# rpng/R-VIO

Measured on AMD Instinct MI355X. Metric: camera frames/sec (KLT+RANSAC track, IMU propagate, MSCKF update, augment/compose), 200 feat / 10-clone window, higher is better.
Workload: dtype f64 (filter) / u8+i32+f32 (KLT); 1 GPU; cfgB: synthetic EuRoC-shaped 752x480 @20Hz, 200 features, 10-clone window, IMU 200 Hz, single stream, equalizer on (CLAHE 3.0, 5x5), corners from the device detector (GFTT + cornerSubPix); parallelism=single GPU

## Files before the change

r-vio_amd/csrc/filter_kernels.hip:

```cpp
#include <type_traits>
#include "rvio_dev.h"
#include "../../include/rvio_hip.h"
#include "solve9.hip"

#include "literal.h"
__device__ const double kChi2Dev[500] = {
#include "chi2_table.inc"
};

typedef double d4 __attribute__((ext_vector_type(4)));

__device__ __forceinline__ double fast_rcp(double v) {
    double y = __builtin_amdgcn_rcp(v);
    y = fma(fma(-v, y, 1.0), y, y);
    return fma(fma(-v, y, 1.0), y, y);
}
__device__ __forceinline__ void sincos_fast(double x, double* sp, double* cp) {
    if (!(fabs(x) < 1e5)) { sincos(x, sp, cp); return; }
    const double kf = rint(x * 6.36619772367581382433e-01);
    double r = fma(-kf, 1.57079632679489655800e+00, x);
    r = fma(-kf, 6.12323399573676603587e-17, r);
    const int q = (int)kf & 3;
    const double z = r * r;
    double ps = fma(z, 1.58969099521155010221e-10, -2.50507602534068634195e-08);
// ... 1712 lines not shown
        for (int u = 0; u < 22; ++u) {
            const int e = tid + u * 256;
            const int rr = e >> 6, k = e & 63;
            if (rr < 88) { Gl[rr * LS + k] = vg[u]; Ul[rr * LS + k] = vu[u]; }
            const int k2 = e / 88, r2 = e - k2 * 88;
            if (k2 < 64) P1c[r2 * LS + k2] = vp[u];
        }
    }
    __syncthreads();
    const int nt = (d + 15) / 16, npair = nt * (nt + 1) / 2;
    const int pr = blockIdx.x * 4 + wave;
    if (pr >= npair) return;
    int I = 0, rem = pr;
    while (rem >= nt - I) { rem -= nt - I; ++I; }
    const int J = I + rem;
    auto xtile = [&](int i0, int j0) -> d4 {
        const int r = i0 + li, c = j0 + li;
        double a1[16], b1[16], p1[4];
#pragma unroll
        for (int q = 0; q < 4; ++q) { const int row = i0 + lk + 4 * q; p1[q] = (row < d && c < d) ? P1[(size_t)row + (size_t)c * ld] : 0.0; }
#pragma unroll
        for (int u = 0; u < 16; ++u) { const int k = 4 * u + lk; a1[u] = (r < d) ? P1c[r * LS + k] : 0.0; b1[u] = (c < d) ? Gl[c * LS + k] : 0.0; }
        d4 acc = {0, 0, 0, 0}, acc2 = {0, 0, 0, 0};
#pragma unroll
        for (int u = 0; u < 16; ++u) acc = __builtin_amdgcn_mfma_f64_16x16x4f64(a1[u], b1[u], acc, 0, 0, 0);
#pragma unroll
        for (int u = 0; u < 16; ++u) { const int k = 4 * u + lk; a1[u] = (r < d) ? Gl[r * LS + k] : 0.0; b1[u] = (c < d) ? Ul[c * LS + k] : 0.0; }
#pragma unroll
        for (int u = 0; u < 16; ++u) acc2 = __builtin_amdgcn_mfma_f64_16x16x4f64(a1[u], b1[u], acc2, 0, 0, 0);
        d4 out;
#pragma unroll
        for (int q = 0; q < 4; ++q) out[q] = p1[q] - acc[q] + s2 * acc2[q];
        return out;
    };
    const d4 xij = xtile(I * 16, J * 16);
    d4 xji = xij;
    if (I != J) xji = xtile(J * 16, I * 16);
#pragma unroll
    for (int q = 0; q < 4; ++q) tl[wave][lk + 4 * q][li] = xji[q];
    __builtin_amdgcn_wave_barrier();
#pragma unroll
    for (int q = 0; q < 4; ++q) {
        const int rr = lk + 4 * q, row = I * 16 + rr, col = J * 16 + li;
        const double v = .5 * (xij[q] + tl[wave][li][rr]);
        if (row < d && col < d) {
            Pout[(size_t)row + (size_t)col * ld] = v;
            if (I != J) Pout[(size_t)col + (size_t)row * ld] = v;
        }
    }
}

#define JL_LS 61
#define JL_LDS_DOUBLES (3 * 60 * JL_LS + 8 * 16 * JL_LS + 16)
__global__ __launch_bounds__(256) void joseph_lds_kernel(DevCfg cfg, int n, const double* __restrict__ P, const double* __restrict__ W, const double* __restrict__ Ab,
                                                         double* __restrict__ Pout, FilterMeta* __restrict__ meta, const double* __restrict__ x, double* __restrict__ x_out,
                                                         const double* __restrict__ dx_scr, int n_pairs, int dx_nt) {
    if (dx_scr && (int)blockIdx.x >= n_pairs) {
        __shared__ S9DxLds dxl;
        s9_dx_role(cfg, meta, n, Ab, x, P, dx_scr, x_out, dx_nt, (int)blockIdx.x - n_pairs, dxl);
        return;
    }
    extern __shared__ __align__(16) double jl[];
    constexpr int LS = JL_LS;
    double* const Wl = jl;
    double* const Al = Wl + 60 * LS;
    double* const Ccl = Al + 60 * LS;
    double* const PcS = Ccl + 60 * LS;
    double* const Us = PcS + 2 * 16 * LS;
    double* const Gs = Us + 2 * 16 * LS;
    double* const Qs = Gs + 2 * 16 * LS;
    constexpr int SS = 16 * LS;
    const int c6 = 6 * n, d = 24 + c6, ldh = cfg.ldh, ld = cfg.dmax;
    const double s2 = cfg.sigma_im * cfg.sigma_im;
    const int tid = threadIdx.x, lane = tid & 63, wave = tid >> 6, li = lane & 15, lk = lane >> 4;
    DBG_R(blockIdx.x == 0, 3);
    const int nt = (d + 15) / 16;
    int I = 0, rem = blockIdx.x;
    while (rem >= nt - I) { rem -= nt - I; ++I; }
    const int J = I + rem;
    const int r0[2] = {I * 16, J * 16};
    auto r0of = [&](int sidx) { return sidx ? J * 16 : I * 16; };
    DBG_T(20);
    double p0[4] = {0, 0, 0, 0}, p0t[4] = {0, 0, 0, 0};
    if (wave == 0) {
#pragma unroll
        for (int q = 0; q < 4; ++q) {
            const int row = r0[0] + lk + 4 * q, c = r0[1] + li;
            const bool ok = row < d && c < d;
            p0[q] = ok ? P[(size_t)row + (size_t)c * ld] : 0.0;
            p0t[q] = ok ? P[(size_t)c + (size_t)row * ld] : 0.0;
        }
    }
    auto ldz = [](const double* __restrict__ p, size_t i, bool ok) { const double v = p[ok ? i : 0]; return ok ? v : 0.0; };
    double vw[15], va[15], vc[15], vs[8];
#pragma unroll
    for (int u = 0; u < 15; ++u) {
        const int e = tid + u * 256, k = e / 60, j = e - k * 60;
        vw[u] = ldz(W, (size_t)k * ldh + j, e < 3600 && k < c6 && j < c6);
    }
#pragma unroll
    for (int u = 0; u < 8; ++u) {
        const int e = tid + u * 256, sidx = e / 960, ee = e - sidx * 960, k = ee >> 4, rr = ee & 15;
        const int row = r0of(sidx & 1) + rr;
        vs[u] = ldz(P, (size_t)row + (size_t)(24 + k) * ld, e < 1920 && k < c6 && row < d);
    }
#pragma unroll
    for (int u = 0; u < 15; ++u) {
        const int e = tid + u * 256, k = e / 60, j = e - k * 60;
        va[u] = ldz(Ab, (size_t)k * ldh + j, e < 3600 && k < c6 && j < c6);
    }
#pragma unroll
    for (int u = 0; u < 15; ++u) {
        const int e = tid + u * 256, k = e / 60, j = e - k * 60;
        vc[u] = ldz(P, (size_t)(24 + j) + (size_t)(24 + k) * ld, e < 3600 && k < c6 && j < c6);
    }
    for (int e = tid; e < 6 * SS; e += 256) Us[e] = 0.0;
#pragma unroll
    for (int u = 0; u < 15; ++u) {
        const int e = tid + u * 256, k = e / 60, j = e - k * 60;
        if (e < 3600) Wl[k * LS + j] = vw[u];
    }
#pragma unroll
    for (int u = 0; u < 8; ++u) {
        const int e = tid + u * 256, sidx = e / 960, ee = e - sidx * 960, k = ee >> 4, rr = ee & 15;
        if (e < 1920) PcS[(sidx & 1) * SS + rr * LS + k] = vs[u];
    }
    __syncthreads();
    DBG_T(21);
    const int ntj = (c6 + 15) / 16;
    auto strips = [&](const double* X, const double* Ym, bool Yt, double* out, const double* sub) {
        const int t0 = wave, t1 = wave + 4, ntile = 2 * ntj;
        const bool v0 = t0 < ntile, v1 = t1 < ntile;
        const int s0 = min(t0 / ntj, 1), c0 = (t0 % ntj) * 16 + li, s1 = min(t1 / ntj, 1), c1 = (t1 % ntj) * 16 + li;
        double a0[15], b0[15], a1[15], b1[15];
#pragma unroll
        for (int u = 0; u < 15; ++u) {
            const int k = 4 * u + lk;
            a0[u] = X[s0 * SS + li * LS + k];
            b0[u] = Yt ? Ym[c0 * LS + k] : Ym[k * LS + c0];
            a1[u] = X[s1 * SS + li * LS + k];
            b1[u] = Yt ? Ym[c1 * LS + k] : Ym[k * LS + c1];
        }
        d4 acc0 = {0, 0, 0, 0}, acc1 = {0, 0, 0, 0};
#pragma unroll
        for (int u = 0; u < 15; ++u) {
            acc0 = __builtin_amdgcn_mfma_f64_16x16x4f64(a0[u], b0[u], acc0, 0, 0, 0);
            acc1 = __builtin_amdgcn_mfma_f64_16x16x4f64(a1[u], b1[u], acc1, 0, 0, 0);
        }
        const bool st0 = v0 && c0 < 60, st1 = v1 && c1 < 60;
#pragma unroll
        for (int q = 0; q < 4; ++q) {
            const int row = lk + 4 * q;
            if (st0) out[s0 * SS + row * LS + c0] = sub ? (sub[s0 * SS + row * LS + min(c0, 59)] - acc0[q]) : acc0[q];
            if (st1) out[s1 * SS + row * LS + c1] = sub ? (sub[s1 * SS + row * LS + min(c1, 59)] - acc1[q]) : acc1[q];
        }
    };
    strips(PcS, Wl, false, Us, nullptr);
#pragma unroll
    for (int u = 0; u < 15; ++u) {
        const int e = tid + u * 256, k = e / 60, j = e - k * 60;
        if (e < 3600) { Al[k * LS + j] = va[u]; Ccl[j * LS + k] = vc[u]; }
    }
    __syncthreads();
    DBG_T(22);
    strips(Us, Al, false, Gs, nullptr);
    __syncthreads();
    DBG_T(23);
    strips(Gs, Ccl, true, Qs, PcS);
    __syncthreads();
    DBG_T(24);
    double (*const xt)[16][17] = reinterpret_cast<double (*)[16][17]>(Wl);
    const int nprod = (I == J) ? 3 : 6;
    auto product = [&](int pidx) -> d4 {
        const int sa = pidx / 3, sb = sa ^ 1, kind = pidx - 3 * sa;
        const double* Xa = (kind == 1 ? Qs : Gs) + sa * SS;
        const double* Yb = (kind == 0 ? PcS : (kind == 1 ? Gs : Us)) + sb * SS;
        double a1[15], b1[15];
#pragma unroll
        for (int u = 0; u < 15; ++u) { const int k = 4 * u + lk; a1[u] = Xa[li * LS + k]; b1[u] = Yb[li * LS + k]; }
        d4 acc = {0, 0, 0, 0};
#pragma unroll
        for (int u = 0; u < 15; ++u) acc = __builtin_amdgcn_mfma_f64_16x16x4f64(a1[u], b1[u], acc, 0, 0, 0);
        return acc;
    };
    {
        const bool two = wave + 4 < nprod;
        d4 pa = {0, 0, 0, 0}, pb = {0, 0, 0, 0};
        if (wave < nprod) pa = product(wave);
        if (two) pb = product(wave + 4);
#pragma unroll
        for (int q = 0; q < 4; ++q) {
            if (wave < nprod) xt[wave][lk + 4 * q][li] = pa[q];
            if (two) xt[wave + 4][lk + 4 * q][li] = pb[q];
        }
    }
    __syncthreads();
    DBG_T(25);
    if (wave == 0) {
        const int o = (I == J) ? 0 : 3;
#pragma unroll
        for (int q = 0; q < 4; ++q) {
            const int rr = lk + 4 * q, row = I * 16 + rr, col = J * 16 + li;
            const double p1 = p0[q] - xt[0][rr][li];
            const double xij = p1 - xt[1][rr][li] + s2 * xt[2][rr][li];
            const double p1t = p0t[q] - xt[o][li][rr];
            const double xji = p1t - xt[o + 1][li][rr] + s2 * xt[o + 2][li][rr];
            const double v = .5 * (xij + xji);
            if (row < d && col < d) {
                Pout[(size_t)row + (size_t)col * ld] = v;
                if (I != J) Pout[(size_t)col + (size_t)row * ld] = v;
            }
        }
    }
}
```

r-vio_amd/csrc/launch_plan.h:

```cpp
#pragma once
#include <stddef.h>

#if defined(__HIPCC__) || defined(__CUDACC__)
#define LP_HD __host__ __device__
#else
#define LP_HD
#endif

#define RVIO_MAX_LEN 32
#define RVIO_MAX_FEATURES 4096
#define GRAM_MAX_FEATS 2048
#define RVIO_LDS_LIMIT 163840
#define LIT_FEATS 24
#define LIT_RING 32
#ifndef FEAT_T_SMALL
#define FEAT_T_SMALL 128
#endif
#define LIT_STAMPS 5
#define LIT_STAMP_OFF 200

LP_HD inline size_t feat_lds_doubles(int max_len, int ldh, bool tm_in_lds) {
    const int L = max_len, M2 = 2 * L, rho = 2 * L - 2;
    size_t n = (size_t)7 * (L - 1) + (size_t)(L - 1) * 24 + L * 6 + M2 * 3 + (L - 1) * 18 + 3 * M2 + 16;
    n += (size_t)M2 * ldh;
    if (tm_in_lds) n += (size_t)rho * ldh;
    n += (size_t)(rho + 1) * (rho + 1);
    return n;
}
LP_HD inline int trunc_mmax(int max_len) { return 6 * ((max_len + 1) / 2 - 1); }
LP_HD inline size_t trunc_lds_doubles(int max_len) { const size_t m = trunc_mmax(max_len); return m * (m | 1) + m + 8; }
LP_HD inline size_t gram_batch_lds_doubles(int max_len, int ldh) {
    const size_t a = (size_t)(ldh - 1) * ldh, t = trunc_lds_doubles(max_len);
    return a > t ? a : t;
}
LP_HD inline size_t lit_tri(int c6) { return (size_t)c6 * (c6 + 1) / 2 + c6; }
LP_HD inline size_t lit_aux_doubles(int ldh, int rho_max) { return (size_t)LIT_RING * ldh + 4 * (size_t)ldh + 2 * 256 + ldh + (size_t)(LIT_FEATS * rho_max + 1) / 2 + 8; }
LP_HD inline size_t lit_state_doubles(int c6) { return 3 * lit_tri(c6); }
LP_HD inline size_t lit_slab_doubles(int ldh, int rho_max) { return (size_t)(rho_max + 2) * (ldh + 3); }
LP_HD inline size_t lit_rows_doubles(int ldh, int rho_max) { return (size_t)LIT_FEATS * (rho_max + 2) * (ldh + 3) + (size_t)LIT_FEATS * rho_max * ldh; }
LP_HD inline size_t book_lds_bytes(int F, int waves) { return (((size_t)20 * F + 7) & ~(size_t)7) + (size_t)waves * F * 8 + 16; }

LP_HD inline size_t lit_norm_off(int ldh) { return (size_t)ldh * ldh; }
LP_HD inline bool lit_stamp_fits(int ldh) { return (size_t)ldh * ldh + LIT_STAMP_OFF + LIT_STAMPS <= 2 * (size_t)ldh * ldh; }
LP_HD inline size_t lit_stamp_off(int ldh, int k) { return (size_t)ldh * ldh + LIT_STAMP_OFF + k; }
LP_HD inline size_t lit_diag_end(int ldh, bool stamps) {
    size_t e = lit_norm_off(ldh) + (size_t)(ldh - 1);
    if (stamps && lit_stamp_fits(ldh)) { const size_t s = lit_stamp_off(ldh, LIT_STAMPS - 1) + 1; if (s > e) e = s; }
    return e;
}

#define LP_S9CHOL4_BYTES 35976
#define LP_S9CHOL6_BYTES 44424
#define LP_S9SMALL_BYTES 160328
#define LP_PROP3_BYTES 86432
#define LP_JB_TL_DOUBLES (12 * 16 * 17)
#define LP_UGL_BYTES ((2 * 64 * 65 + 88 * 65 + 2 * 16 * 65) * 8)
#define LP_FNL_BYTES ((3 * 88 * 65 + 4 * 16 * 17) * 8)
#define LP_JL_BYTES ((3 * 60 * 61 + 8 * 16 * 61 + 16) * 8)
#define LP_GEMM_T_LDS_BYTES (2 * 64 * 65 * 8)

enum LpKernel {
    LPK_FEAT_BUILD16, LPK_FEAT_BUILD4, LPK_GRAM_REDUCE, LPK_BLOCK_SUM, LPK_LIT_BATCH, LPK_GEMM_T_LDS, LPK_GRAM_BATCH4, LPK_GRAM_BATCH6, LPK_FEAT_PROP,
    LPK_BOOKKEEP_B, LPK_RANSAC_BOOK, LPK_SOLVE9_SMALL, LPK_SOLVE6_1, LPK_SOLVE6_2, LPK_SOLVE6_3, LPK_JOSEPH_BATCH, LPK_UG, LPK_UG_LDS, LPK_FINAL_LDS,
    LPK_JOSEPH_LDS, LPK_COUNT
};
static const char* const kLpKernelName[LPK_COUNT] = {
    "feat_build_kernel<16>", "feat_build_kernel<4>", "gram_reduce_kernel", "block_sum_kernel", "lit_batch_kernel", "gemm_T_lds_kernel",
    "gram_reduce_batch_kernel<4>", "gram_reduce_batch_kernel<6>", "feat_prop_kernel", "bookkeep_b_kernel", "ransac_book_kernel", "solve9_small_kernel",
    "solve6_kernel<1, 8, 8>", "solve6_kernel<2, 12, 8>", "solve6_kernel<2, 16, 8>", "joseph_batch_kernel", "ug_kernel", "ug_lds_kernel", "final_lds_kernel",
    "joseph_lds_kernel"
};

struct LaunchPlan {
    int rc = 0;
    const char* why = nullptr;
    int Fu = 0, ldh = 0, rho_max = 0;
    int feat_threads = 256;
    int n_ic = 2;
    bool chol_queue = false;
    size_t trunc_lds = 0, lit_batch_lds = 0, feat_lds = 0, fprop_lds = 0, gram_batch_lds = 0, book_lds = 0, solve5_lds = 0, jb_lds = 0, ug_lds = 0;
    bool lit_state_global = false, tm_global = false, fuse_ok = false;
    bool lit_ok = false;
    int book_waves = 4;
    bool book_fused = false;
    int solve5_variant = 0, solve7_variant = 0, solve9_nt = 0;
    size_t attr[LPK_COUNT] = {};
};

LP_HD inline size_t lp_max(size_t a, size_t b) { return a > b ? a : b; }
LP_HD inline size_t lp_min(size_t a, size_t b) { return a < b ? a : b; }

inline LaunchPlan launch_plan(int max_len, int n_features, int batch, const size_t* statics) {
    LaunchPlan p;
    const int nmax = max_len - 1;
    p.Fu = (n_features + 1) / 2; p.ldh = 6 * nmax + 1; p.rho_max = 2 * max_len - 2;
    const size_t ldh = p.ldh, c6m = ldh - 1;
    const int F = n_features;
    if (max_len < 3 || max_len > RVIO_MAX_LEN || n_features < 2 || batch < 1) { p.rc = 1; p.why = "invalid configuration"; return p; }
    if (p.Fu > GRAM_MAX_FEATS) { p.rc = 1; p.why = "Tracker.nFeatures too large: at most 4096 (RVIO_MAX_FEATURES; ceil(F/2) hand-over slots <= 2048 in the Gram stage)"; return p; }
    if (batch == 1 && c6m > 96 && c6m <= 192) { p.n_ic = 1; p.chol_queue = true; }
    p.feat_threads = (p.ldh <= 128) ? FEAT_T_SMALL : 256;
    p.lit_ok = p.ldh <= 190 && nmax + 1 <= 40 && p.rho_max < 254 && lit_slab_doubles(p.ldh, p.rho_max) * sizeof(double) <= 144 * 1024;
    p.trunc_lds = trunc_lds_doubles(max_len) * sizeof(double);
    {
        const size_t aux = lit_aux_doubles(p.ldh, p.rho_max) * sizeof(double), st = lit_state_doubles(p.ldh - 1) * sizeof(double);
        const size_t slab = lit_slab_doubles(p.ldh, p.rho_max) * sizeof(double);
        p.lit_state_global = batch > 1 || aux + st > 144 * 1024;
        p.lit_batch_lds = lp_max(aux, slab);
        p.trunc_lds = lp_max(p.trunc_lds, lp_max(p.lit_state_global ? aux : aux + st, lp_min((size_t)4, (size_t)(144 * 1024) / slab) * slab));
    }
    p.feat_lds = feat_lds_doubles(max_len, p.ldh, true) * sizeof(double);
// ... 364 lines not shown
```

r-vio_amd/csrc/rvio_hip.hip:

```cpp
#include <hip/hip_runtime.h>
#include <atomic>
#include <chrono>
#include <dlfcn.h>
#include <cmath>
#include <cstdio>
#include <cstdlib>
#include <cstring>
#include <map>
#include <mutex>
#include <string>
#include <vector>

#include "../../include/rvio_hip.h"
#include "rvio_dev.h"
#include "frontend_dev.h"
#include "filter_kernels.hip"
#include "filter_kernels2.hip"
#include "solve6.hip"
#include "solve7.hip"
#include "solve9.hip"
#include "landmarks.hip"
#include "odom.hip"
#pragma clang fp contract(off)
#include "frontend_kernels.hip"
// ... 827 lines not shown
    if (NT == 8) hipLaunchKernelGGL((solve9_chol_kernel<2, 4>), dim3(1), dim3(1024), 0, st, h->dc, n, Pc, h->S9scr);
    else hipLaunchKernelGGL((solve9_chol_kernel<3, 4>), dim3(1), dim3(1024), 0, st, h->dc, n, Pc, h->S9scr);
}
static void launch_s9_sweep(rvio_hip* h, int NT, const double* Ab) {
    if (NT == 8) hipLaunchKernelGGL((solve9_sweep_kernel<2, 4>), dim3(1), dim3(1024), 0, h->stream, h->dc, Ab, h->S9scr);
    else hipLaunchKernelGGL((solve9_sweep_kernel<3, 4>), dim3(1), dim3(1024), 0, h->stream, h->dc, Ab, h->S9scr);
}
static bool take_chol(rvio_hip* h) {
    if (h->chol_async && hipStreamWaitEvent(h->stream, h->evL, 0) != hipSuccess) { h->chol_async = false; h->chol_ready = false; }
    const bool pre = h->chol_ready || h->chol_async;
    h->chol_ready = false; h->chol_async = false;
    return pre;
}

static void launch_solve(rvio_hip* h, const UpdateForms& f, int n, const double* Ab) {
    const DevCfg& d = h->dc;
    double *xin = h->x[h->cur], *xout = h->x[h->cur ^ 1], *Pc = h->P[h->cur];
    const dim3 gb(1, 1, h->batch);
    const size_t bs = h->slab_bytes;
    const bool roles = f.dx == LPD_ROLES;
    switch (f.solve) {
    case LPS_NONE: break;
    case LPS_SMALL: hipLaunchKernelGGL(solve9_small_kernel, dim3(1), dim3(1024), f.solve_lds.bytes, h->stream, d, h->meta, n, Ab, xin, Pc, h->S9scr, h->W, xout, roles ? h->S9scr + S9_YP_OFF(4) : (double*)nullptr); break;
    case LPS_S9_1_4: hipLaunchKernelGGL((solve9_kernel<1, 4>), gb, dim3(1024), 0, h->stream, d, h->meta, n, Ab, xin, Pc, h->S9scr, h->W, xout, bs, (size_t)0); break;
    case LPS_S9_2_3_PRE: hipLaunchKernelGGL((solve9_kernel<2, 3, true>), gb, dim3(576), 0, h->stream, d, h->meta, n, Ab, xin, Pc, h->S9scr, h->W, xout, bs, (size_t)0, roles ? 1 : 0); break;
    case LPS_S9_2_3: hipLaunchKernelGGL((solve9_kernel<2, 3>), gb, dim3(576), 0, h->stream, d, h->meta, n, Ab, xin, Pc, h->S9scr, h->W, xout, bs, (size_t)0, roles ? 1 : 0); break;
    case LPS_SPLIT: {
        const int NT = f.split_nt, nwg = (NT * NT + 3) / 4;
        if (f.own_chol) launch_s9_chol(h, NT, n, Pc, h->stream);
        hipLaunchKernelGGL(solve9_prod_kernel<0>, dim3(nwg), dim3(256), 0, h->stream, d, n, Ab, h->S9scr, h->W, NT);
        hipLaunchKernelGGL(solve9_prod_kernel<1>, dim3(nwg), dim3(256), 0, h->stream, d, n, Ab, h->S9scr, h->W, NT);
        launch_s9_sweep(h, NT, Ab);
        hipLaunchKernelGGL(solve9_prod_kernel<2>, dim3(nwg), dim3(256), 0, h->stream, d, n, Ab, h->S9scr, h->W, NT);
        hipLaunchKernelGGL(solve9_prod_kernel<3>, dim3(nwg), dim3(256), 0, h->stream, d, n, Ab, h->S9scr, h->W, NT);
        if (f.dx == LPD_KERNEL) hipLaunchKernelGGL(solve9_dx_kernel, dim3(1), dim3(1024), 0, h->stream, d, h->meta, n, Ab, xin, Pc, h->S9scr, h->W, xout, NT);
        break;
    }
    case LPS_SOLVE7: hipLaunchKernelGGL((solve7_kernel<3, 16, 12>), gb, dim3(768), 0, h->stream, d, h->meta, n, Ab, xin, Pc, h->Tbuf, h->W, xout, bs); break;
    case LPS_SOLVE6_1: hipLaunchKernelGGL((solve6_kernel<1, 8, 8>), gb, dim3(512), f.solve_lds.bytes, h->stream, d, h->meta, n, h->Tbuf, Ab, xin, Pc, h->W, xout, bs); break;
    case LPS_SOLVE6_2: hipLaunchKernelGGL((solve6_kernel<2, 12, 8>), gb, dim3(512), f.solve_lds.bytes, h->stream, d, h->meta, n, h->Tbuf, Ab, xin, Pc, h->W, xout, bs); break;
    case LPS_SOLVE6_3: hipLaunchKernelGGL((solve6_kernel<2, 16, 8>), gb, dim3(512), f.solve_lds.bytes, h->stream, d, h->meta, n, h->Tbuf, Ab, xin, Pc, h->W, xout, bs); break;
    }
}

static void launch_ug_final(rvio_hip* h, const UpdateForms& f, int n, const double* Ab, double* Pn, bool ug, bool fin, bool roles) {
    const DevCfg& d = h->dc;
    const int B = h->batch;
    const size_t bs = h->slab_bytes;
    double* Pc = h->P[h->cur];
    const int role_wgs = roles ? f.role_wgs : 0;
    const double *nod = nullptr, *yp = role_wgs ? (const double*)h->S9scr : nod;
    switch (f.joseph) {
    case LPJ_BATCH: hipLaunchKernelGGL(joseph_batch_kernel, dim3(1, 1, B), dim3(JB_THREADS), f.ug_lds.bytes, h->stream, d, n, Pc, h->W, Ab, Pn, bs); break;
    case LPJ_LDS: hipLaunchKernelGGL(joseph_lds_kernel, dim3(f.grid[0] + role_wgs), dim3(256), f.ug_lds.bytes, h->stream, d, n, Pc, h->W, Ab, Pn, h->meta, (const double*)h->x[h->cur], h->x[h->cur ^ 1], yp, f.grid[0], h->plan.solve9_nt); break;
    case LPJ_LDS_PAIR:
        if (ug) hipLaunchKernelGGL(ug_lds_kernel, dim3(f.grid[0]), dim3(256), f.ug_lds.bytes, h->stream, d, n, Pc, h->W, Ab, h->U, h->G, h->Pt1);
        if (fin) hipLaunchKernelGGL(final_lds_kernel, dim3(f.grid[1]), dim3(256), f.fin_lds.bytes, h->stream, d, n, h->Pt1, h->G, h->U, Pn);
        break;
    case LPJ_TILE:
        if (ug) {
            hipLaunchKernelGGL(ug_tile_kernel<0>, dim3(f.grid[0] + role_wgs), dim3(256), 0, h->stream, d, n, Pc, h->W, Ab, h->U, h->G, h->Pt1,
                               h->meta, (const double*)h->x[h->cur], h->x[h->cur ^ 1], yp, h->plan.solve9_nt);
            hipLaunchKernelGGL(ug_tile_kernel<1>, dim3(f.grid[1]), dim3(256), 0, h->stream, d, n, Pc, h->W, Ab, h->U, h->G, h->Pt1, h->meta, nod, (double*)nullptr, nod, 0);
            hipLaunchKernelGGL(ug_tile_kernel<2>, dim3(f.grid[2]), dim3(256), 0, h->stream, d, n, Pc, h->W, Ab, h->U, h->G, h->Pt1, h->meta, nod, (double*)nullptr, nod, 0);
        }
        if (fin) hipLaunchKernelGGL(final_tile_kernel, dim3(f.grid[3]), dim3(256), 0, h->stream, d, n, h->Pt1, h->G, h->U, Pn);
        break;
    case LPJ_STRIPS:
        if (ug) hipLaunchKernelGGL(ug_kernel, dim3(f.grid[0], 1, B), dim3(256), f.ug_lds.bytes, h->stream, d, n, Pc, h->W, Ab, h->U, h->G, h->Pt1, bs);
        if (fin) hipLaunchKernelGGL(final_kernel, dim3(f.grid[1], 1, B), dim3(256), 0, h->stream, d, n, h->Pt1, h->G, h->U, Pn, bs);
        break;
    }
}

static void launch_landmarks(rvio_hip* h, int n, const LmOut& out) {
    const int T = std::min(LM_MAX_T, 64 * ((h->dc.Fu + 63) / 64));
    hipLaunchKernelGGL(landmark_kernel, dim3(1, 1, h->batch), dim3(T), 0, h->stream, h->dc, n, (const double*)h->x[h->cur ^ 1], (const double*)h->x[h->cur],
                       (const int*)h->t.n_feat, (const unsigned char*)h->t.types, (const int*)h->t.len, (const int*)h->acc, (const double*)h->pfinv,
                       h->slab_bytes, h->bin, out, (const CamCal*)h->cal);
}
static dim3 lp_grid(const LpLaunch& l) { return dim3((unsigned)l.gx, (unsigned)l.gy, (unsigned)l.gz); }
static dim3 lp_block(const LpLaunch& l) { return dim3((unsigned)l.threads); }
static void launch_subpix(rvio_hip* h, const FrontForms& f, const DetDev& q, const uint8_t* img, int stride, size_t src_bs, int frame, hipStream_t st) {
    const size_t bs = h->slab_bytes;
    const LpLaunch& l = f.subpix_l;
    switch (f.subpix) {
    case LPSP_NONE: break;
    case LPSP_WIDE_WIN: hipLaunchKernelGGL(subpix_wide_kernel, lp_grid(l), lp_block(l), l.lds, st, img, stride, q, src_bs, bs); break;
    case LPSP_GENERIC: hipLaunchKernelGGL(subpix_generic_kernel, lp_grid(l), lp_block(l), 0, st, img, stride, q, src_bs, bs); break;
    case LPSP_X16: hipLaunchKernelGGL(subpix_kernel16, lp_grid(l), lp_block(l), 0, st, img, stride, q, src_bs, bs); break;
    case LPSP_STOCK: hipLaunchKernelGGL(subpix_kernel, lp_grid(l), lp_block(l), 0, st, img, stride, q, src_bs, bs, frame); break;
    }
}
static int lm_alloc(rvio_hip* h, LmOut* out) {
    const size_t Fu = (size_t)h->dc.Fu;
    auto up = [](size_t b) { return (b + 255) & ~(size_t)255; };
    const size_t o_feat = 256, o_pr = o_feat + up(sizeof(int) * Fu), o_pw = o_pr + up(sizeof(double) * 3 * Fu), bs = o_pw + up(sizeof(double) * 3 * Fu);
    char* p = nullptr;
    HIPCHK(h, hipMalloc((void**)&p, bs * h->batch));
    h->allocs.push_back(p);
    HIPCHK(h, hipMemsetAsync(p, 0, bs * h->batch, h->stream));
    *out = LmOut{(int*)p, (int*)(p + o_feat), (double*)(p + o_pr), (double*)(p + o_pw), bs};
    return RVIO_OK;
}

static int update_global_dev(rvio_hip* h, const double* d_blocks, int world, bool combined) {
    const DevCfg& d = h->dc;
// ... 1300 lines not shown
```

r-vio_amd/csrc/solve9.hip:

```cpp
#pragma once
#include "rvio_dev.h"

typedef double s9_d4 __attribute__((ext_vector_type(4)));
#define S9_TILE 256

__device__ __forceinline__ bool lane_is(int li, int lk, int a, int b) { return li == a && lk == b; }
struct S9Wave {
    double rowb[2][128];
    double tb[16 * 17 + 64 + 192];
};
typedef __attribute__((address_space(3))) double s9_lds_t;
typedef volatile s9_lds_t* s9_vlp;

__device__ __forceinline__ s9_d4 s9_tn(const s9_d4& x, const s9_d4& y, s9_d4 acc) {
    acc = __builtin_amdgcn_mfma_f64_16x16x4f64(x[0], y[0], acc, 0, 0, 0);
    acc = __builtin_amdgcn_mfma_f64_16x16x4f64(x[1], y[1], acc, 0, 0, 0);
    acc = __builtin_amdgcn_mfma_f64_16x16x4f64(x[2], y[2], acc, 0, 0, 0);
    acc = __builtin_amdgcn_mfma_f64_16x16x4f64(x[3], y[3], acc, 0, 0, 0);
    return acc;
}
__device__ __forceinline__ s9_d4 s9_zero() { s9_d4 z = {0.0, 0.0, 0.0, 0.0}; return z; }
__device__ __forceinline__ s9_d4 s9_ldg(const double* t, int lane) {
    s9_d4 v = {t[lane], t[64 + lane], t[128 + lane], t[192 + lane]};
    return v;
}
__device__ __forceinline__ void s9_stg(double* t, int lane, const s9_d4& v) {
    t[lane] = v[0]; t[64 + lane] = v[1]; t[128 + lane] = v[2]; t[192 + lane] = v[3];
}
__device__ __forceinline__ s9_d4 s9_lds(const double* t_, int lane) {
    const s9_lds_t* t = (const s9_lds_t*)t_;
    s9_d4 v = {t[lane], t[64 + lane], t[128 + lane], t[192 + lane]};
    return v;
}
__device__ __forceinline__ void s9_sts(double* t_, int lane, const s9_d4& v) {
    s9_lds_t* t = (s9_lds_t*)t_;
    t[lane] = v[0]; t[64 + lane] = v[1]; t[128 + lane] = v[2]; t[192 + lane] = v[3];
}
__device__ __forceinline__ s9_d4 s9_transpose_tb(const s9_d4& v, double* tb_, int li, int lk) {
    s9_vlp tb = (s9_vlp)tb_;
#pragma unroll
    for (int r = 0; r < 4; ++r) tb[(4 * r + lk) * 17 + li] = v[r];
    s9_d4 t;
#pragma unroll
    for (int r = 0; r < 4; ++r) t[r] = tb[li * 17 + 4 * r + lk];
    return t;
}

__device__ __forceinline__ double s9_rsqrt(double t) {
    double y = __builtin_amdgcn_rsq(t);
    const double h = 0.5 * t;
    y = fma(y, fma(-(h * y), y, 0.5), y);
    y = fma(y, fma(-(h * y), y, 0.5), y);
    return y;
}
__device__ __forceinline__ void s9_factor(s9_d4 m, const double* ref_, double tol, S9Wave* ws, int li, int lk, s9_d4& F, s9_d4& Ft, int& bad) {
    const s9_lds_t* ref = (const s9_lds_t*)ref_;
    const int lane = li + 16 * lk;
    s9_d4 e;
#pragma unroll
    for (int r = 0; r < 4; ++r) e[r] = (4 * r + lk == li) ? 1.0 : 0.0;
#pragma unroll
    for (int b = 0; b < 4; ++b) {
        s9_vlp rb = (s9_vlp)ws->rowb[b & 1];
        rb[lane] = m[b];
        rb[64 + lane] = e[b];
        const double a00 = rb[0 * 16 + 4 * b + 0];
        const double a10 = rb[1 * 16 + 4 * b + 0], a11 = rb[1 * 16 + 4 * b + 1];
        const double a20 = rb[2 * 16 + 4 * b + 0], a21 = rb[2 * 16 + 4 * b + 1], a22 = rb[2 * 16 + 4 * b + 2];
        const double a30 = rb[3 * 16 + 4 * b + 0], a31 = rb[3 * 16 + 4 * b + 1], a32 = rb[3 * 16 + 4 * b + 2], a33 = rb[3 * 16 + 4 * b + 3];
        double Rv[4], Ev[4];
#pragma unroll
        for (int v = 0; v < 4; ++v) { Rv[v] = rb[v * 16 + li]; Ev[v] = rb[64 + v * 16 + li]; }
        double lim[4];
#pragma unroll
        for (int k = 0; k < 4; ++k) lim[k] = ref_ ? tol * ref[4 * b + k] : 0.0;
        auto pivot = [&](double t, int k) {
            const bool ok = t > lim[k] && t > 0.0;
            if (!ok && (ref_ == nullptr || !(t >= -lim[k]))) bad |= 1;
            return ok ? s9_rsqrt(t) : 0.0;
        };
        const double i0 = pivot(a00, 0);
        const double l10 = a10 * i0, l20 = a20 * i0, l30 = a30 * i0;
        const double i1 = pivot(fma(-l10, l10, a11), 1);
        const double l21 = fma(-l20, l10, a21) * i1, l31 = fma(-l30, l10, a31) * i1;
        const double i2 = pivot(fma(-l21, l21, fma(-l20, l20, a22)), 2);
        const double l32 = fma(-l31, l21, fma(-l30, l20, a32)) * i2;
        const double i3 = pivot(fma(-l32, l32, fma(-l31, l31, fma(-l30, l30, a33))), 3);
        const double f00 = i0, f11 = i1, f22 = i2, f33 = i3;
        const double f10 = -(l10 * f00) * i1;
        const double f21 = -(l21 * f11) * i2;
        const double f32 = -(l32 * f22) * i3;
        const double f20 = -fma(l21, f10, l20 * f00) * i2;
        const double f31 = -fma(l32, f21, l31 * f11) * i3;
        const double f30 = -fma(l32, f20, fma(l31, f10, l30 * f00)) * i3;
        const double g0 = lk == 0 ? f00 : lk == 1 ? f10 : lk == 2 ? f20 : f30;
        const double g1 = lk == 0 ? 0.0 : lk == 1 ? f11 : lk == 2 ? f21 : f31;
        const double g2 = lk <= 1 ? 0.0 : lk == 2 ? f22 : f32;
        const double g3 = lk == 3 ? f33 : 0.0;
        const double z = fma(g3, Rv[3], fma(g2, Rv[2], fma(g1, Rv[1], g0 * Rv[0])));
        const double ze = fma(g3, Ev[3], fma(g2, Ev[2], fma(g1, Ev[1], g0 * Ev[0])));
        const double za = (li > 4 * b + 3) ? -z : 0.0;
        m = __builtin_amdgcn_mfma_f64_16x16x4f64(za, z, m, 0, 0, 0);
        e = __builtin_amdgcn_mfma_f64_16x16x4f64(za, ze, e, 0, 0, 0);
        e[b] = ze;
    }
    F = e;
    Ft = s9_transpose_tb(F, ws->tb, li, lk);
}

template <class FX, class FY>
__device__ __forceinline__ s9_d4 s9_gemm(int k0, int k1, FX fx, FY fy) {
    s9_d4 acc = s9_zero();
    if (k0 >= k1) return acc;
    s9_d4 xa = fx(k0), xb = fy(k0);
#pragma unroll 2
    for (int k = k0; k < k1; ++k) {
        s9_d4 na = xa, nb = xb;
        if (k + 1 < k1) { na = fx(k + 1); nb = fy(k + 1); }
        acc = s9_tn(xa, xb, acc);
        xa = na; xb = nb;
    }
    return acc;
// ... 576 lines not shown
    S9Wave ws;
    double b[64], y[64], yp[4][64];
    double dx[24 + 64];
    double part[4 * (24 + 64)];
    int bad;
};
__global__ __launch_bounds__(1024) void solve9_small_kernel(DevCfg cfg, FilterMeta* __restrict__ meta, int n, const double* __restrict__ Ab,
                                                            const double* __restrict__ x, const double* __restrict__ P, const double* __restrict__ scr,
                                                            double* __restrict__ Wout, double* __restrict__ x_out, double* __restrict__ yp_out) {
    constexpr int NT = 4, NTH = 1024;
    extern __shared__ __align__(16) double s9s_dyn[];
    S9SmallLds& sh = *reinterpret_cast<S9SmallLds*>(s9s_dyn);
    const int c6 = 6 * n, d = 24 + c6, ldh = cfg.ldh, ld = cfg.dmax, xd = 26 + 7 * n;
    const int tid = threadIdx.x, lane = tid & 63, wv = __builtin_amdgcn_readfirstlane(tid >> 6), li = lane & 15, lk = lane >> 4;
    const int ti = wv >> 2, tj = wv & 3;
    const int n_good = (int)Ab[(size_t)ldh * (ldh - 1)], n_rows = (int)Ab[(size_t)ldh * (ldh - 1) + 1];
    const bool upd = n_good > 2;
    DBG_R(true, 2);
    if (tid == 0) { meta->n_good = n_good; meta->n_rows = n_rows; meta->updated = upd ? 1 : 0; meta->trunc_at = (int)Ab[(size_t)ldh * (ldh - 1) + 2]; sh.bad = 0; }
    if (!upd) {
        for (int e = tid; e < c6 * c6; e += NTH) Wout[(size_t)(e / c6) * ldh + (e % c6)] = 0.0;
        if (!yp_out) for (int i = tid; i < xd; i += NTH) x_out[i] = x[i];
        return;
    }
    DBG_T(30);
    const double s2 = cfg.sigma_im * cfg.sigma_im;
    auto ld_A = [&](int i, int j) {
        s9_d4 v;
#pragma unroll
        for (int r = 0; r < 4; ++r) {
            const int row = 16 * i + 4 * r + lk, col = 16 * j + li;
            v[r] = (row < c6 && col < c6) ? Ab[(size_t)row * ldh + col] : 0.0;
        }
        return v;
    };
    const s9_d4 a0 = ld_A(ti, tj);
    const bool lowt = ti >= tj;
    s9_d4 l0 = s9_zero(), g0 = s9_zero();
    if (lowt) { l0 = s9_ldg(scr + (size_t)(ti * NT + tj) * S9_TILE, lane); g0 = s9_ldg(scr + (size_t)NT * NT * S9_TILE + (size_t)(tj * NT + ti) * S9_TILE, lane); }
    constexpr int PCN = (88 * 64 + NTH - 1) / NTH;
    double pc[PCN];
#pragma unroll
    for (int u = 0; u < PCN; ++u) {
        const int e = tid + u * NTH, k = e / 88, i = e - k * 88;
        pc[u] = (!yp_out && k < c6 && i < d) ? P[(size_t)i + (size_t)(24 + k) * ld] : 0.0;
    }
    if (tid < 64) sh.b[tid] = (tid < c6) ? Ab[(size_t)tid * ldh + c6] : 0.0;
    if (tid == 0 && scr[(size_t)5 * NT * NT * S9_TILE] != 0.0) sh.bad = 1;
    if (lowt) { s9_sts(sh.L[ti * NT + tj], lane, l0); s9_sts(sh.G[ti * (ti + 1) / 2 + tj], lane, g0); }
    s9_sts(sh.Q[wv], lane, a0);
    __syncthreads();
    DBG_T(32);
    {
        s9_d4 q = s9_zero(), rr = s9_zero();
#pragma unroll
        for (int k = 0; k < NT; ++k) {
            if (k >= tj) q = s9_tn(s9_lds(sh.Q[k * NT + ti], lane), s9_lds(sh.L[k * NT + tj], lane), q);
            if (k >= ti) rr = s9_tn(s9_lds(sh.L[k * NT + ti], lane), s9_lds(sh.Q[k * NT + tj], lane), rr);
        }
        __syncthreads();
        s9_sts(sh.Q[wv], lane, q);
        s9_sts(sh.R[wv], lane, rr);
    }
    __syncthreads();
    DBG_T(33);
    s9_d4 S = s9_zero();
#pragma unroll
    for (int k = 0; k < NT; ++k)
        if (k >= ti) S = s9_tn(s9_lds(sh.L[k * NT + ti], lane), s9_lds(sh.Q[k * NT + tj], lane), S);
    if (ti == tj) {
#pragma unroll
        for (int r = 0; r < 4; ++r) if (4 * r + lk == li) S[r] += s2;
    }
    DBG_T(34);
    int bad = 0;
#pragma unroll 1
    for (int k = 0; k < NT; ++k) {
        double (*rowp)[S9_TILE] = sh.rowp[k & 1];
        if (ti == k) s9_sts(rowp[tj], lane, S);
        __syncthreads();
        s9_d4 F, Ft;
        if (wv == 0) {
            s9_factor(s9_lds(rowp[k], lane), nullptr, 0.0, &sh.ws, li, lk, F, Ft, bad);
            s9_sts(sh.F[0], lane, F);
            s9_sts(sh.F[1], lane, Ft);
        }
        __syncthreads();
        F = s9_lds(sh.F[0], lane);
        if (wv < NT) {
            Ft = s9_lds(sh.F[1], lane);
            s9_sts(sh.Z[wv], lane, s9_tn(Ft, s9_lds(rowp[wv], lane), s9_zero()));
        }
        __syncthreads();
        if (ti == k && tj == k) {
            const s9_d4 dd = s9_tn(F, F, s9_zero());
#pragma unroll
            for (int r = 0; r < 4; ++r) S[r] = -dd[r];
        } else if (ti == k) S = s9_tn(F, s9_lds(sh.Z[tj], lane), s9_zero());
        else if (tj == k) S = s9_tn(s9_lds(sh.Z[ti], lane), F, s9_zero());
        else {
            const s9_d4 Zr = s9_lds(sh.Z[ti], lane);
            s9_d4 nz;
#pragma unroll
            for (int r = 0; r < 4; ++r) nz[r] = -Zr[r];
            S = s9_tn(nz, s9_lds(sh.Z[tj], lane), S);
        }
    }
    {
        s9_d4 v;
#pragma unroll
        for (int r = 0; r < 4; ++r) v[r] = -S[r];
        s9_sts(sh.Q[wv], lane, v);
    }
    __syncthreads();
    DBG_T(35);
    {
        s9_d4 v = s9_zero();
#pragma unroll
        for (int k = 0; k < NT; ++k) v = s9_tn(s9_lds(sh.Q[k * NT + ti], lane), s9_lds(sh.R[k * NT + tj], lane), v);
        s9_sts(sh.L[wv], lane, v);
    }
    __syncthreads();
    DBG_T(36);
    double* pcs = &sh.Q[0][0];
    if (!yp_out) {
#pragma unroll
        for (int u = 0; u < PCN; ++u) { const int e = tid + u * NTH; if (e < 88 * 64) ((s9_lds_t*)pcs)[e] = pc[u]; }
    }
    {
        const double is2 = 1.0 / s2;
        s9_d4 acc = s9_zero();
#pragma unroll
        for (int k = 0; k < NT; ++k)
            if (k <= ti) acc = s9_tn(s9_lds(sh.G[ti * (ti + 1) / 2 + k], lane), s9_lds(sh.L[k * NT + tj], lane), acc);
        double t = 0.0;
#pragma unroll
        for (int r = 0; r < 4; ++r) {
            const int a = 16 * ti + 4 * r + lk, bcol = 16 * tj + li;
            const double w = (((a == bcol) ? 1.0 : 0.0) - acc[r]) * is2;
            if (a < c6 && bcol < c6) Wout[(size_t)bcol * ldh + a] = w;
            t = fma(w, sh.b[a], t);
        }
        t += __shfl_xor(t, 16); t += __shfl_xor(t, 32);
// ... 43 lines not shown
```

Before: 11050 frames/s.

## Widen Joseph LDS kernel to 512 threads and trim solve9 small-kernel syncs

```diff
diff --git a/r-vio_amd/csrc/filter_kernels.hip b/r-vio_amd/csrc/filter_kernels.hip
--- a/r-vio_amd/csrc/filter_kernels.hip
+++ b/r-vio_amd/csrc/filter_kernels.hip
@@ -1788,7 +1788,7 @@
 
 #define JL_LS 61
 #define JL_LDS_DOUBLES (3 * 60 * JL_LS + 8 * 16 * JL_LS + 16)
-__global__ __launch_bounds__(256) void joseph_lds_kernel(DevCfg cfg, int n, const double* __restrict__ P, const double* __restrict__ W, const double* __restrict__ Ab,
+__global__ __launch_bounds__(LP_JL_THREADS) void joseph_lds_kernel(DevCfg cfg, int n, const double* __restrict__ P, const double* __restrict__ W, const double* __restrict__ Ab,
                                                          double* __restrict__ Pout, FilterMeta* __restrict__ meta, const double* __restrict__ x, double* __restrict__ x_out,
                                                          const double* __restrict__ dx_scr, int n_pairs, int dx_nt) {
     if (dx_scr && (int)blockIdx.x >= n_pairs) {
@@ -1797,7 +1797,7 @@
         return;
     }
     extern __shared__ __align__(16) double jl[];
-    constexpr int LS = JL_LS;
+    constexpr int LS = JL_LS, NTH = LP_JL_THREADS;
     double* const Wl = jl;
     double* const Al = Wl + 60 * LS;
     double* const Ccl = Al + 60 * LS;
@@ -1828,73 +1828,67 @@
         }
     }
     auto ldz = [](const double* __restrict__ p, size_t i, bool ok) { const double v = p[ok ? i : 0]; return ok ? v : 0.0; };
-    double vw[15], va[15], vc[15], vs[8];
-#pragma unroll
-    for (int u = 0; u < 15; ++u) {
-        const int e = tid + u * 256, k = e / 60, j = e - k * 60;
+    double vw[8], va[8], vc[8], vs[4];
+#pragma unroll
+    for (int u = 0; u < 8; ++u) {
+        const int e = tid + u * NTH, k = e / 60, j = e - k * 60;
         vw[u] = ldz(W, (size_t)k * ldh + j, e < 3600 && k < c6 && j < c6);
     }
 #pragma unroll
-    for (int u = 0; u < 8; ++u) {
-        const int e = tid + u * 256, sidx = e / 960, ee = e - sidx * 960, k = ee >> 4, rr = ee & 15;
+    for (int u = 0; u < 4; ++u) {
+        const int e = tid + u * NTH, sidx = e / 960, ee = e - sidx * 960, k = ee >> 4, rr = ee & 15;
         const int row = r0of(sidx & 1) + rr;
         vs[u] = ldz(P, (size_t)row + (size_t)(24 + k) * ld, e < 1920 && k < c6 && row < d);
     }
 #pragma unroll
-    for (int u = 0; u < 15; ++u) {
-        const int e = tid + u * 256, k = e / 60, j = e - k * 60;
+    for (int u = 0; u < 8; ++u) {
+        const int e = tid + u * NTH, k = e / 60, j = e - k * 60;
         va[u] = ldz(Ab, (size_t)k * ldh + j, e < 3600 && k < c6 && j < c6);
     }
 #pragma unroll
-    for (int u = 0; u < 15; ++u) {
-        const int e = tid + u * 256, k = e / 60, j = e - k * 60;
+    for (int u = 0; u < 8; ++u) {
+        const int e = tid + u * NTH, k = e / 60, j = e - k * 60;
         vc[u] = ldz(P, (size_t)(24 + j) + (size_t)(24 + k) * ld, e < 3600 && k < c6 && j < c6);
     }
-    for (int e = tid; e < 6 * SS; e += 256) Us[e] = 0.0;
-#pragma unroll
-    for (int u = 0; u < 15; ++u) {
-        const int e = tid + u * 256, k = e / 60, j = e - k * 60;
+    for (int e = tid; e < 6 * SS; e += NTH) Us[e] = 0.0;
+#pragma unroll
+    for (int u = 0; u < 8; ++u) {
+        const int e = tid + u * NTH, k = e / 60, j = e - k * 60;
         if (e < 3600) Wl[k * LS + j] = vw[u];
     }
 #pragma unroll
-    for (int u = 0; u < 8; ++u) {
-        const int e = tid + u * 256, sidx = e / 960, ee = e - sidx * 960, k = ee >> 4, rr = ee & 15;
+    for (int u = 0; u < 4; ++u) {
+        const int e = tid + u * NTH, sidx = e / 960, ee = e - sidx * 960, k = ee >> 4, rr = ee & 15;
         if (e < 1920) PcS[(sidx & 1) * SS + rr * LS + k] = vs[u];
     }
     __syncthreads();
     DBG_T(21);
     const int ntj = (c6 + 15) / 16;
     auto strips = [&](const double* X, const double* Ym, bool Yt, double* out, const double* sub) {
-        const int t0 = wave, t1 = wave + 4, ntile = 2 * ntj;
-        const bool v0 = t0 < ntile, v1 = t1 < ntile;
-        const int s0 = min(t0 / ntj, 1), c0 = (t0 % ntj) * 16 + li, s1 = min(t1 / ntj, 1), c1 = (t1 % ntj) * 16 + li;
-        double a0[15], b0[15], a1[15], b1[15];
+        const int t0 = wave, ntile = 2 * ntj;
+        const bool v0 = t0 < ntile;
+        const int s0 = min(t0 / ntj, 1), c0 = (t0 % ntj) * 16 + li;
+        double a0[15], b0[15];
 #pragma unroll
         for (int u = 0; u < 15; ++u) {
             const int k = 4 * u + lk;
             a0[u] = X[s0 * SS + li * LS + k];
             b0[u] = Yt ? Ym[c0 * LS + k] : Ym[k * LS + c0];
-            a1[u] = X[s1 * SS + li * LS + k];
-            b1[u] = Yt ? Ym[c1 * LS + k] : Ym[k * LS + c1];
-        }
-        d4 acc0 = {0, 0, 0, 0}, acc1 = {0, 0, 0, 0};
-#pragma unroll
-        for (int u = 0; u < 15; ++u) {
-            acc0 = __builtin_amdgcn_mfma_f64_16x16x4f64(a0[u], b0[u], acc0, 0, 0, 0);
-            acc1 = __builtin_amdgcn_mfma_f64_16x16x4f64(a1[u], b1[u], acc1, 0, 0, 0);
-        }
-        const bool st0 = v0 && c0 < 60, st1 = v1 && c1 < 60;
+        }
+        d4 acc0 = {0, 0, 0, 0};
+#pragma unroll
+        for (int u = 0; u < 15; ++u) acc0 = __builtin_amdgcn_mfma_f64_16x16x4f64(a0[u], b0[u], acc0, 0, 0, 0);
+        const bool st0 = v0 && c0 < 60;
 #pragma unroll
         for (int q = 0; q < 4; ++q) {
             const int row = lk + 4 * q;
             if (st0) out[s0 * SS + row * LS + c0] = sub ? (sub[s0 * SS + row * LS + min(c0, 59)] - acc0[q]) : acc0[q];
-            if (st1) out[s1 * SS + row * LS + c1] = sub ? (sub[s1 * SS + row * LS + min(c1, 59)] - acc1[q]) : acc1[q];
         }
     };
     strips(PcS, Wl, false, Us, nullptr);
 #pragma unroll
-    for (int u = 0; u < 15; ++u) {
-        const int e = tid + u * 256, k = e / 60, j = e - k * 60;
+    for (int u = 0; u < 8; ++u) {
+        const int e = tid + u * NTH, k = e / 60, j = e - k * 60;
         if (e < 3600) { Al[k * LS + j] = va[u]; Ccl[j * LS + k] = vc[u]; }
     }
     __syncthreads();
@@ -1919,16 +1913,10 @@
         for (int u = 0; u < 15; ++u) acc = __builtin_amdgcn_mfma_f64_16x16x4f64(a1[u], b1[u], acc, 0, 0, 0);
         return acc;
     };
-    {
-        const bool two = wave + 4 < nprod;
-        d4 pa = {0, 0, 0, 0}, pb = {0, 0, 0, 0};
-        if (wave < nprod) pa = product(wave);
-        if (two) pb = product(wave + 4);
-#pragma unroll
-        for (int q = 0; q < 4; ++q) {
-            if (wave < nprod) xt[wave][lk + 4 * q][li] = pa[q];
-            if (two) xt[wave + 4][lk + 4 * q][li] = pb[q];
-        }
+    if (wave < nprod) {
+        const d4 pa = product(wave);
+#pragma unroll
+        for (int q = 0; q < 4; ++q) xt[wave][lk + 4 * q][li] = pa[q];
     }
     __syncthreads();
     DBG_T(25);
diff --git a/r-vio_amd/csrc/launch_plan.h b/r-vio_amd/csrc/launch_plan.h
--- a/r-vio_amd/csrc/launch_plan.h
+++ b/r-vio_amd/csrc/launch_plan.h
@@ -52,11 +52,13 @@
 #define LP_S9CHOL4_BYTES 35976
 #define LP_S9CHOL6_BYTES 44424
 #define LP_S9SMALL_BYTES 160328
+#define LP_S9SMALL_QR_MAP 0xAEBF9D7C68235410ull
 #define LP_PROP3_BYTES 86432
 #define LP_JB_TL_DOUBLES (12 * 16 * 17)
 #define LP_UGL_BYTES ((2 * 64 * 65 + 88 * 65 + 2 * 16 * 65) * 8)
 #define LP_FNL_BYTES ((3 * 88 * 65 + 4 * 16 * 17) * 8)
 #define LP_JL_BYTES ((3 * 60 * 61 + 8 * 16 * 61 + 16) * 8)
+#define LP_JL_THREADS 512
 #define LP_GEMM_T_LDS_BYTES (2 * 64 * 65 * 8)
 
 enum LpKernel {
diff --git a/r-vio_amd/csrc/rvio_hip.hip b/r-vio_amd/csrc/rvio_hip.hip
--- a/r-vio_amd/csrc/rvio_hip.hip
+++ b/r-vio_amd/csrc/rvio_hip.hip
@@ -903,7 +903,7 @@
     const double *nod = nullptr, *yp = role_wgs ? (const double*)h->S9scr : nod;
     switch (f.joseph) {
     case LPJ_BATCH: hipLaunchKernelGGL(joseph_batch_kernel, dim3(1, 1, B), dim3(JB_THREADS), f.ug_lds.bytes, h->stream, d, n, Pc, h->W, Ab, Pn, bs); break;
-    case LPJ_LDS: hipLaunchKernelGGL(joseph_lds_kernel, dim3(f.grid[0] + role_wgs), dim3(256), f.ug_lds.bytes, h->stream, d, n, Pc, h->W, Ab, Pn, h->meta, (const double*)h->x[h->cur], h->x[h->cur ^ 1], yp, f.grid[0], h->plan.solve9_nt); break;
+    case LPJ_LDS: hipLaunchKernelGGL(joseph_lds_kernel, dim3(f.grid[0] + role_wgs), dim3(LP_JL_THREADS), f.ug_lds.bytes, h->stream, d, n, Pc, h->W, Ab, Pn, h->meta, (const double*)h->x[h->cur], h->x[h->cur ^ 1], yp, f.grid[0], h->plan.solve9_nt); break;
     case LPJ_LDS_PAIR:
         if (ug) hipLaunchKernelGGL(ug_lds_kernel, dim3(f.grid[0]), dim3(256), f.ug_lds.bytes, h->stream, d, n, Pc, h->W, Ab, h->U, h->G, h->Pt1);
         if (fin) hipLaunchKernelGGL(final_lds_kernel, dim3(f.grid[1]), dim3(256), f.fin_lds.bytes, h->stream, d, n, h->Pt1, h->G, h->U, Pn);
diff --git a/r-vio_amd/csrc/solve9.hip b/r-vio_amd/csrc/solve9.hip
--- a/r-vio_amd/csrc/solve9.hip
+++ b/r-vio_amd/csrc/solve9.hip
@@ -64,10 +64,11 @@
         s9_vlp rb = (s9_vlp)ws->rowb[b & 1];
         rb[lane] = m[b];
         rb[64 + lane] = e[b];
-        const double a00 = rb[0 * 16 + 4 * b + 0];
-        const double a10 = rb[1 * 16 + 4 * b + 0], a11 = rb[1 * 16 + 4 * b + 1];
-        const double a20 = rb[2 * 16 + 4 * b + 0], a21 = rb[2 * 16 + 4 * b + 1], a22 = rb[2 * 16 + 4 * b + 2];
-        const double a30 = rb[3 * 16 + 4 * b + 0], a31 = rb[3 * 16 + 4 * b + 1], a32 = rb[3 * 16 + 4 * b + 2], a33 = rb[3 * 16 + 4 * b + 3];
+        auto piv = [&](int i, int j) { return readlane_f64(m[b], 16 * i + 4 * b + j); };
+        const double a00 = piv(0, 0);
+        const double a10 = piv(1, 0), a11 = piv(1, 1);
+        const double a20 = piv(2, 0), a21 = piv(2, 1), a22 = piv(2, 2);
+        const double a30 = piv(3, 0), a31 = piv(3, 1), a32 = piv(3, 2), a33 = piv(3, 3);
         double Rv[4], Ev[4];
 #pragma unroll
         for (int v = 0; v < 4; ++v) { Rv[v] = rb[v * 16 + li]; Ev[v] = rb[64 + v * 16 + li]; }
@@ -750,15 +751,16 @@
     __syncthreads();
     DBG_T(32);
     {
+        const int qt = (int)((LP_S9SMALL_QR_MAP >> (4 * wv)) & 15), qi = qt >> 2, qj = qt & 3;
         s9_d4 q = s9_zero(), rr = s9_zero();
 #pragma unroll
         for (int k = 0; k < NT; ++k) {
-            if (k >= tj) q = s9_tn(s9_lds(sh.Q[k * NT + ti], lane), s9_lds(sh.L[k * NT + tj], lane), q);
-            if (k >= ti) rr = s9_tn(s9_lds(sh.L[k * NT + ti], lane), s9_lds(sh.Q[k * NT + tj], lane), rr);
-        }
-        __syncthreads();
-        s9_sts(sh.Q[wv], lane, q);
-        s9_sts(sh.R[wv], lane, rr);
+            if (k >= qj) q = s9_tn(s9_lds(sh.Q[k * NT + qi], lane), s9_lds(sh.L[k * NT + qj], lane), q);
+            if (k >= qi) rr = s9_tn(s9_lds(sh.L[k * NT + qi], lane), s9_lds(sh.Q[k * NT + qj], lane), rr);
+        }
+        __syncthreads();
+        s9_sts(sh.Q[qt], lane, q);
+        s9_sts(sh.R[qt], lane, rr);
     }
     __syncthreads();
     DBG_T(33);
@@ -775,18 +777,18 @@
 #pragma unroll 1
     for (int k = 0; k < NT; ++k) {
         double (*rowp)[S9_TILE] = sh.rowp[k & 1];
-        if (ti == k) s9_sts(rowp[tj], lane, S);
-        __syncthreads();
-        s9_d4 F, Ft;
-        if (wv == 0) {
-            s9_factor(s9_lds(rowp[k], lane), nullptr, 0.0, &sh.ws, li, lk, F, Ft, bad);
-            s9_sts(sh.F[0], lane, F);
-            s9_sts(sh.F[1], lane, Ft);
-        }
-        __syncthreads();
-        F = s9_lds(sh.F[0], lane);
-        if (wv < NT) {
-            Ft = s9_lds(sh.F[1], lane);
+        if (ti == k) {
+            if (tj == k) {
+                s9_d4 F, Ft;
+                s9_factor(S, nullptr, 0.0, &sh.ws, li, lk, F, Ft, bad);
+                s9_sts(sh.F[0], lane, F);
+                s9_sts(sh.F[1], lane, Ft);
+            } else s9_sts(rowp[tj], lane, S);
+        }
+        __syncthreads();
+        const s9_d4 F = s9_lds(sh.F[0], lane);
+        if (wv < NT && wv != k) {
+            const s9_d4 Ft = s9_lds(sh.F[1], lane);
             s9_sts(sh.Z[wv], lane, s9_tn(Ft, s9_lds(rowp[wv], lane), s9_zero()));
         }
         __syncthreads();
```

Result: faster. 11310 frames/s (median of 6 runs) (+2.4%).
